# edwardyehuang/iSeg

Hardware: AMD Instinct MI355X
Metric: train_images_per_sec (ConvNeXt-T+ASPP 512x512 crop, fwd+bwd+AdamW, whole job) (higher is better)
Workload: dtype bf16

## Files before the change

### include/iseg_hip.h

```cpp
#ifndef ISEG_HIP_H
#define ISEG_HIP_H

#include <stddef.h>
#include <stdint.h>

#ifdef __cplusplus
extern "C" {
#endif

#ifndef ISEG_HIP_STREAM_T
#define ISEG_HIP_STREAM_T
typedef struct ihipStream_t* iseg_stream_t;
#endif

#define ISEG_STATUS_OK 0
#define ISEG_STATUS_ARG (-1)
#define ISEG_STATUS_HIP (-2)
#define ISEG_STATUS_UNSUPPORTED (-3)
#define ISEG_STATUS_WORKSPACE (-4)

#define ISEG_DTYPE_F32 0
#define ISEG_DTYPE_BF16 1

#define ISEG_ACT_NONE 0
// ... 484 lines not shown
int iseg_convnext_weight_prep_batched(const int64_t* table, int entries, int64_t max_elements, iseg_stream_t stream);
int iseg_convnext_mlp_fwd(const void* y2, const void* fw_tiled, const float* b1, const float* b2, const float* gamma,
                          const float* rowscale, int64_t rows_per_group, const void* residual, void* out, int64_t M, int C, int dtype,
                          iseg_stream_t stream);
int iseg_convnext_mlp_bwd(const void* y2, const void* dbr, const void* bw_tiled, const float* b1, void* g, void* dh, void* dy2,
                          int64_t M, int C, int dtype, iseg_stream_t stream);
int iseg_convnext_mlp_bwd_data(const void* y, const float* mean, const float* rstd, const float* ln_gamma, const float* ln_beta,
                               const void* dout, const float* rowscale, int64_t rows_per_group, const void* bw_tiled, const float* b1,
                               void* dy2, int64_t M, int C, int dtype, iseg_stream_t stream);

size_t iseg_convnext_mlp_bwd_data_ln_workspace_bytes(int64_t M, int C);
int iseg_convnext_mlp_bwd_data_ln(const void* y1, const float* mean, const float* rstd, const float* ln_gamma, const float* ln_beta,
                                  const void* dout, const float* rowscale, int64_t rows_per_group, const void* bw_tiled, const float* b1,
                                  void* dy1, float* dln_gamma, float* dln_beta, int64_t M, int C, int dtype, void* ws, size_t ws_bytes,
                                  iseg_stream_t stream);
int iseg_convnext_mlp_fwd_ln(const void* y1, const float* ln_gamma, const float* ln_beta, float eps, float* mean, float* rstd,
                             const void* fw_tiled, const float* b1, const float* b2, const float* gamma, const float* rowscale,
                             int64_t rows_per_group, const void* residual, void* out, int64_t M, int C, int dtype, iseg_stream_t stream);
size_t iseg_convnext_mlp_wgrad_workspace_bytes(int64_t M, int C);
int iseg_convnext_mlp_wgrad(const void* y, const float* mean, const float* rstd, const float* ln_gamma, const float* ln_beta,
                            const void* dout, const float* rowscale, int64_t rows_per_group, const void* bw_tiled, const float* b1,
                            const float* W2, const float* b2, const float* gamma, float* dW1, float* db1, float* dW2, float* db2,
                            float* dgamma, int64_t M, int C, int dtype, void* ws, size_t ws_bytes, iseg_stream_t stream);

#ifdef __cplusplus
}
#endif
#endif
```

### iseg_amd/_hip.py

```python
import ctypes as C
import os

_HERE = os.path.dirname(os.path.abspath(__file__))
LIB_PATH = os.path.join(_HERE, "lib", "libiseg_hip.so")

F32, BF16 = 0, 1
ACT_NONE, ACT_RELU, ACT_GELU, ACT_GELU_GRAD, ACT_RELU_GRAD, ACT_MUL_AUX, ACT_SIGMOID, ACT_SWISH = 0, 1, 2, 3, 4, 5, 6, 7


class HipLibraryMissing(RuntimeError):
    pass


class HipCallError(RuntimeError):
    pass


class GemmArgs(C.Structure):
    _fields_ = [
        ("A", C.c_void_p), ("lda", C.c_int64), ("a_kcontig", C.c_int),
        ("B", C.c_void_p), ("ldb", C.c_int64), ("b_kcontig", C.c_int),
        ("D", C.c_void_p), ("ldd", C.c_int64),
        ("M", C.c_int64), ("N", C.c_int64), ("K", C.c_int64),
        ("in_dtype", C.c_int), ("out_dtype", C.c_int),
# ... 233 lines not shown
    "iseg_conv2d_patch_fwd": (_i, [_p, _p, _p, _p, C.POINTER(ConvGeom), _i, _p, _z, _p]),
    "iseg_conv2d_patch_bwd_data": (_i, [_p, _p, _p, C.POINTER(ConvGeom), _i, _p, _z, _p]),
    "iseg_conv2d_patch_bwd_weight": (_i, [_p, _p, _p, _p, _i, C.POINTER(ConvGeom), _i, _p, _z, _p]),
    "iseg_conv2d_branches_supported": (_i, [C.POINTER(ConvBranches), _i]),
    "iseg_conv2d_branches_fwd": (_i, [_p, C.POINTER(ConvBranches), _i, _p, _z, _p]),
    "iseg_conv2d_branches_bwd_data": (_i, [C.POINTER(ConvBranches), _p, _p, _l, _i, _p, _z, _p]),
    "iseg_conv2d_branches_bwd_weight": (_i, [_p, C.POINTER(ConvBranches), _i, _i, _p, _z, _p]),
    "iseg_convnext_mlp_supported": (_i, [_i, _i]),
    "iseg_convnext_mlp_tiled_bytes": (_z, [_i, _i]),
    "iseg_convnext_mlp_prep": (_i, [_p, _p, _p, _p, _p, _i, _p]),
    "iseg_convnext_mlp_fwd": (_i, [_p, _p, _p, _p, _p, _p, _l, _p, _p, _l, _i, _i, _p]),
    "iseg_convnext_mlp_bwd": (_i, [_p, _p, _p, _p, _p, _p, _p, _l, _i, _i, _p]),
    "iseg_convnext_mlp_bwd_data": (_i, [_p, _p, _p, _p, _p, _p, _p, _l, _p, _p, _p, _l, _i, _i, _p]),
    "iseg_convnext_mlp_bwd_data_ln_workspace_bytes": (_z, [_l, _i]),
    "iseg_convnext_mlp_bwd_data_ln": (_i, [_p, _p, _p, _p, _p, _p, _p, _l, _p, _p, _p, _p, _p, _l, _i, _i, _p, _z, _p]),
    "iseg_convnext_weight_prep_batched": (_i, [_p, _i, _l, _p]),
    "iseg_convnext_mlp_fwd_ln": (_i, [_p, _p, _p, _f, _p, _p, _p, _p, _p, _p, _p, _l, _p, _p, _l, _i, _i, _p]),
    "iseg_convnext_mlp_wgrad_workspace_bytes": (_z, [_l, _i]),
    "iseg_convnext_mlp_wgrad": (_i, [_p, _p, _p, _p, _p, _p, _p, _l, _p, _p, _p, _p, _p, _p, _p, _p, _p, _p, _l, _i, _i, _p, _z, _p]),
    "iseg_sgd_momentum_step": (_i, [_p, _p, _p, _p, _p, _p, _p, _p, _f, _i, _p, _f, _p, _f, _l, _p]),
}

_lib = None


def lib():
    global _lib
    if _lib is None:
        if not os.path.exists(LIB_PATH):
            raise HipLibraryMissing(
# ... 27 lines not shown
```

### iseg_amd/csrc/mlp_fused.hip

```cpp
#include "common.h"
#include "iseg_hip.h"
#include "mlp_common.h"
#include <stdlib.h>

namespace {

typedef __attribute__((ext_vector_type(16))) float f32x16;
typedef __attribute__((address_space(3))) void* lds_void_ptr;
typedef const __attribute__((address_space(1))) void* glb_void_ptr;

constexpr int OUT_SLAB = 32 * 36 * 4;

template <int C, int SUB, int WAVES, int NIMG, int NSTAGES> struct MlpGeom {
    static constexpr int NS = NSTAGES;
    static constexpr int HID = 4 * C, KK = C / 16, CB = C / 32;
    static constexpr int IMG = C * 64;
    static constexpr int SLAB = NIMG * IMG;
    static constexpr int STAGE = SUB * SLAB;
    static constexpr int PIECES = STAGE / 1024;
    static constexpr int PLO = PIECES / WAVES, NHI = PIECES % WAVES, PHI = PLO + (NHI ? 1 : 0);
    static constexpr int NST = HID / (32 * SUB);
    static constexpr int RING = NS * STAGE > WAVES * OUT_SLAB ? NS * STAGE : WAVES * OUT_SLAB;
    static constexpr int LDS = RING + HID * 4;
    static_assert(C % 32 == 0 && STAGE % 1024 == 0 && HID % (32 * SUB) == 0 && PLO >= 1 && NST >= NS - 1 && NS >= 2 && LDS <= 160 * 1024, "geometry");
// ... 184 lines not shown
        for (int w = 0; w < 2; ++w) {
            auto sw = __builtin_amdgcn_permlane32_swap(d[4 * pr + w], d[4 * pr + 2 + w], false, false);
            d[4 * pr + w] = sw[0];
            d[4 * pr + 2 + w] = sw[1];
        }
    p0 = make_uint4(d[0], d[1], d[2], d[3]);
    p1 = make_uint4(d[4], d[5], d[6], d[7]);
}

template <int C, int SUB, int WAVES, int NSTAGES, bool STORE, bool LNB = false>
__global__ __launch_bounds__(64 * WAVES) void convnext_mlp_bwd_kernel(const bf16_t* __restrict__ Y, const bf16_t* __restrict__ D,
                                                                      const float* __restrict__ rowscale, int64_t rows_per_group,
                                                                      const void* __restrict__ BW, const float* __restrict__ b1,
                                                                      bf16_t* __restrict__ Gout, bf16_t* __restrict__ DHout,
                                                                      bf16_t* __restrict__ DY, int64_t M, MlpLayerNorm ln,
                                                                      float* __restrict__ ln_partials) {
    using G = MlpGeom<C, SUB, WAVES, 3, NSTAGES>;
    constexpr int HID = G::HID, KK = G::KK, CB = G::CB, IMG = G::IMG, SLAB = G::SLAB, STAGE = G::STAGE, NST = G::NST, NS = G::NS;
    constexpr int STORES = STORE ? 4 * SUB : 0;
    extern __shared__ __attribute__((aligned(1024))) char smem[];
    float* const b1s = reinterpret_cast<float*>(smem + G::RING);

    const int tid = threadIdx.x, lane = tid & 63, wid = tid >> 6;
    const int r = lane & 31, h = lane >> 5;
    const int64_t m0 = (int64_t)blockIdx.x * (32 * WAVES) + wid * 32;
    const bool active = m0 < M;

    bf16x8 yf[KK], df[KK];
    {
        int64_t row = m0 + r;
        row = row < M ? row : M - 1;
// ... 163 lines not shown
        }
    } else {
        float* const lnacc = reinterpret_cast<float*>(smem + WAVES * OUT_SLAB);
        float* const gam_s = lnacc + WAVES * 2 * C;
        const int64_t mr = m < M ? m : M - 1;
        bf16x8 yraw[CB][2];
#pragma unroll
        for (int cb = 0; cb < CB; ++cb) {
            yraw[cb][0] = *reinterpret_cast<const bf16x8*>(Y + mr * C + 32 * cb + 16 * eh);
            yraw[cb][1] = *reinterpret_cast<const bf16x8*>(Y + mr * C + 32 * cb + 16 * eh + 8);
        }
        const float mean = ln.mean[mr], rstd = ln.rstd[mr];
        for (int i = tid; i < WAVES * 2 * C; i += 64 * WAVES) lnacc[i] = 0.f;
        for (int i = tid; i < C; i += 64 * WAVES) gam_s[i] = ln.gamma[i];
        __syncthreads();
        const bool live = active && m < M;
        float s1 = 0.f, s2 = 0.f;
        auto xhat16 = [&](int cb, float* xh) {
#pragma unroll
            for (int u = 0; u < 8; ++u) {
                xh[u] = ((float)yraw[cb][0][u] - mean) * rstd;
                xh[8 + u] = ((float)yraw[cb][1][u] - mean) * rstd;
            }
        };
        auto gamma16 = [&](int c0, float* gm) {
#pragma unroll
            for (int i = 0; i < 4; ++i) {
                const float4 t = *reinterpret_cast<const float4*>(gam_s + c0 + 4 * i);
                gm[4 * i] = t.x, gm[4 * i + 1] = t.y, gm[4 * i + 2] = t.z, gm[4 * i + 3] = t.w;
            }
// ... 125 lines not shown
                   int64_t rows_per_group, const void* residual, void* out, int64_t M, const MlpLayerNorm& ln, hipStream_t s) {
    using G = MlpGeom<C, SUB, WAVES, 2, NSTAGES>;
    static const bool raised = [] {
        return hipFuncSetAttribute(reinterpret_cast<const void*>(&convnext_mlp_fwd_kernel<C, SUB, WAVES, NSTAGES>),
                                   hipFuncAttributeMaxDynamicSharedMemorySize, G::LDS) == hipSuccess;
    }();
    (void)raised;
    const int grid = (int)ceil_div64(M, 32 * WAVES);
    hipLaunchKernelGGL((convnext_mlp_fwd_kernel<C, SUB, WAVES, NSTAGES>), dim3(grid), dim3(64 * WAVES), G::LDS, s, (const bf16_t*)y2, FW, b1, b2, gamma, rowscale,
                       rows_per_group, (const bf16_t*)residual, (bf16_t*)out, M, ln);
    return iseg_check_launch("iseg_convnext_mlp_fwd");
}

template <int C, int SUB, int WAVES, int NSTAGES, bool STORE, bool LNB = false>
int launch_mlp_bwd(const void* y2, const void* dbr, const float* rowscale, int64_t rows_per_group, const void* BW, const float* b1, void* g,
                   void* dh, void* dy2, int64_t M, const MlpLayerNorm& ln, hipStream_t s, float* ln_partials = nullptr) {
    using G = MlpGeom<C, SUB, WAVES, 3, NSTAGES>;
    static_assert(!LNB || G::RING >= WAVES * OUT_SLAB + (WAVES * 2 + 1) * C * 4, "the column sums and gamma sit behind the epilogue slabs inside the ring");
    static const bool raised = [] {
        return hipFuncSetAttribute(reinterpret_cast<const void*>(&convnext_mlp_bwd_kernel<C, SUB, WAVES, NSTAGES, STORE, LNB>),
                                   hipFuncAttributeMaxDynamicSharedMemorySize, G::LDS) == hipSuccess;
    }();
    (void)raised;
    const int grid = (int)ceil_div64(M, 32 * WAVES);
    hipLaunchKernelGGL((convnext_mlp_bwd_kernel<C, SUB, WAVES, NSTAGES, STORE, LNB>), dim3(grid), dim3(64 * WAVES), G::LDS, s, (const bf16_t*)y2,
                       (const bf16_t*)dbr, rowscale, rows_per_group, BW, b1, (bf16_t*)g, (bf16_t*)dh, (bf16_t*)dy2, M, ln, ln_partials);
    return iseg_check_launch("iseg_convnext_mlp_bwd");
}

}

extern "C" int iseg_convnext_mlp_supported(int C, int dtype) {
    return dtype == ISEG_BF16 && (C == 96 || C == 192) ? 1 : 0;
}

extern "C" size_t iseg_convnext_mlp_tiled_bytes(int C, int backward) { return (size_t)(backward ? 3 : 2) * 4 * C * C * 2; }

extern "C" int iseg_convnext_mlp_prep(const float* W1, const float* W2, const float* gamma, void* fw_tiled, void* bw_tiled, int C,
                                      hipStream_t stream) {
    ISEG_REQUIRE(W1 && W2 && fw_tiled && C > 0 && C % 32 == 0, "iseg_convnext_mlp_prep: bad arguments");
    const int total = (bw_tiled ? 5 : 2) * 4 * C * C;
// ... 57 lines not shown
    ISEG_REQUIRE((((uintptr_t)y2 | (uintptr_t)dout | (uintptr_t)bw_tiled | (uintptr_t)b1 | (uintptr_t)dy2) & 15) == 0,
                 "iseg_convnext_mlp_bwd_data: operands must be 16-byte aligned");
    ISEG_REQUIRE(!mean || (rstd && ln_gamma && ln_beta && (((uintptr_t)ln_gamma | (uintptr_t)ln_beta) & 15) == 0),
                 "iseg_convnext_mlp_bwd_data: mean needs rstd and 16-byte aligned ln_gamma / ln_beta");
    const MlpLayerNorm ln{mean ? ln_gamma : nullptr, ln_beta, const_cast<float*>(mean), const_cast<float*>(rstd), 0.f};
    if (C == 96) return launch_mlp_bwd<96, 2, 8, 3, false>(y2, dout, rowscale, rows_per_group, bw_tiled, b1, nullptr, nullptr, dy2, M, ln, stream);
    return launch_mlp_bwd<192, 1, 4, 3, false>(y2, dout, rowscale, rows_per_group, bw_tiled, b1, nullptr, nullptr, dy2, M, ln, stream);
}

static int64_t mlp_bwd_blocks(int64_t M, int C) { return ceil_div64(M, 32 * (C == 96 ? 8 : 4)); }

extern "C" size_t iseg_convnext_mlp_bwd_data_ln_workspace_bytes(int64_t M, int C) {
    return (C == 96 || C == 192) && M > 0 ? (size_t)mlp_bwd_blocks(M, C) * 2 * C * sizeof(float) : 0;
}

extern "C" int iseg_convnext_mlp_bwd_data_ln(const void* y1, const float* mean, const float* rstd, const float* ln_gamma, const float* ln_beta,
                                             const void* dout, const float* rowscale, int64_t rows_per_group, const void* bw_tiled,
                                             const float* b1, void* dy1, float* dln_gamma, float* dln_beta, int64_t M, int C, int dtype,
                                             void* ws, size_t ws_bytes, hipStream_t stream) {
    ISEG_REQUIRE(dtype == ISEG_BF16 && (C == 96 || C == 192), "iseg_convnext_mlp_bwd_data_ln: bf16 storage with C = 96 or 192 only (C = %d, dtype = %d)", C, dtype);
    ISEG_REQUIRE(y1 && mean && rstd && ln_gamma && ln_beta && dout && bw_tiled && b1 && dy1 && dln_gamma && dln_beta && M > 0,
                 "iseg_convnext_mlp_bwd_data_ln: null operand or empty problem");
    ISEG_REQUIRE(!rowscale || rows_per_group > 0, "iseg_convnext_mlp_bwd_data_ln: rowscale needs rows_per_group > 0");
    ISEG_REQUIRE((((uintptr_t)y1 | (uintptr_t)dout | (uintptr_t)bw_tiled | (uintptr_t)b1 | (uintptr_t)dy1 | (uintptr_t)ln_gamma | (uintptr_t)ln_beta) & 15) == 0,
                 "iseg_convnext_mlp_bwd_data_ln: operands must be 16-byte aligned");
    const size_t need = iseg_convnext_mlp_bwd_data_ln_workspace_bytes(M, C);
    ISEG_NEED_WORKSPACE("iseg_convnext_mlp_bwd_data_ln", ws, ws_bytes, need);
    const MlpLayerNorm ln{ln_gamma, ln_beta, const_cast<float*>(mean), const_cast<float*>(rstd), 0.f};
    float* partials = (float*)ws;
    float* const arena = iseg_deferred_partials(need, dln_gamma, dln_beta, 1, stream);
    if (arena) partials = arena;
    const int rc = C == 96 ? launch_mlp_bwd<96, 2, 8, 3, false, true>(y1, dout, rowscale, rows_per_group, bw_tiled, b1, nullptr, nullptr, dy1, M, ln,
                                                                       stream, partials)
                           : launch_mlp_bwd<192, 1, 4, 3, false, true>(y1, dout, rowscale, rows_per_group, bw_tiled, b1, nullptr, nullptr, dy1, M, ln,
                                                                        stream, partials);
    if (rc != ISEG_OK) return rc;
    const int blocks = (int)mlp_bwd_blocks(M, C);
    if (arena) iseg_deferred_push(partials, blocks, 2 * C, 2 * C, dln_gamma, dln_beta, C, 1.f, stream);
    else launch_reduce_rows(partials, blocks, 2 * C, 0, 1, 2 * C, dln_gamma, dln_beta, C, 0, 1.f, 1, stream);
    return iseg_check_launch("iseg_convnext_mlp_bwd_data_ln");
}
```

### iseg_amd/csrc/mlp_wgrad.hip

```cpp
#include "common.h"
#include "iseg_hip.h"
#include "mlp_common.h"

namespace {

typedef __attribute__((address_space(3))) bf16x4* lds_bf16x4_ptr;

template <int C> struct WgGeom {
    static constexpr int WAVES = 8, NT = 64 * WAVES, RT = C > 96 ? 32 : 64;
    static constexpr int HID = 4 * C, KS = C / 32, CBS = C / 16;
    static constexpr int NHG = HID / (16 * WAVES);
    static constexpr int STRIDE = (((2 * C + 223) / 256) * 256 + 32) / 2;
    static constexpr int TILE = RT * STRIDE;
    static constexpr int CPR = C / 8;
    static constexpr int RG = (NT / CPR) >= 32 ? 32 : 16;
    static constexpr int NLOAD = CPR * RG, RPT = RT / RG;
    static constexpr int LDS = 2 * 2 * TILE * 2;
    static constexpr int IMG = C * 64, SLAB = 3 * IMG;
    static_assert(C % 32 == 0 && HID % (16 * WAVES) == 0 && NLOAD <= NT && RT % RG == 0 && LDS <= 160 * 1024, "geometry");
};

__device__ __forceinline__ f32x4 mfma16(const bf16x8& a, const bf16x8& b, const f32x4& c) {
    return __builtin_amdgcn_mfma_f32_16x16x32_bf16(a, b, c, 0, 0, 0);
}

__device__ __forceinline__ bf16x8 tr_frag(const bf16_t* rows, int stride, int cb, int lane) {
    const int q = lane >> 4, qq = (lane >> 2) & 3, p = lane & 3;
    const bf16_t* a0 = rows + (4 * q + qq) * stride + 16 * cb + 4 * p;
    const bf16x4 lo = __builtin_amdgcn_ds_read_tr16_b64_v4bf16((lds_bf16x4_ptr)(a0));
    const bf16x4 hi = __builtin_amdgcn_ds_read_tr16_b64_v4bf16((lds_bf16x4_ptr)(a0 + 16 * stride));
    bf16x8 f;
#pragma unroll
    for (int i = 0; i < 4; ++i) {
        f[i] = lo[i];
        f[4 + i] = hi[i];
    }
    return f;
}

template <int C>
__global__ __launch_bounds__(512) void convnext_mlp_wgrad_kernel(const bf16_t* __restrict__ Y, const float* __restrict__ mean,
                                                                 const float* __restrict__ rstd, const float* __restrict__ ln_gamma,
                                                                 const float* __restrict__ ln_beta, const bf16_t* __restrict__ D,
                                                                 const float* __restrict__ rowscale, int64_t rows_per_group,
                                                                 const void* __restrict__ BW, const float* __restrict__ b1,
                                                                 float* __restrict__ part, int64_t M, int64_t rows_per_chunk, int nchunk) {
    using G = WgGeom<C>;
    constexpr int HID = G::HID, KS = G::KS, CBS = G::CBS, STRIDE = G::STRIDE, TILE = G::TILE, RT = G::RT, RG = G::RG, RPT = G::RPT, CPR = G::CPR;
    extern __shared__ __attribute__((aligned(16))) char smem[];
    bf16_t* const tiles = reinterpret_cast<bf16_t*>(smem);

    const int wg = blockIdx.x, xcd = wg & 7, idx = wg >> 3;
    const int hg = idx % G::NHG, chunk = (idx / G::NHG) * 8 + xcd;
    if (chunk >= nchunk) return;
    const int tid = threadIdx.x, lane = tid & 63, wid = tid >> 6;
    const int li = lane & 15, q = lane >> 4;
    const int hid0 = (hg * G::WAVES + wid) * 16;
    const int64_t r_begin = (int64_t)chunk * rows_per_chunk;
    const int64_t r_end = r_begin + rows_per_chunk < M ? r_begin + rows_per_chunk : M;
    const int ntiles = (int)((r_end - r_begin + RT - 1) / RT);

    bf16x8 w1f[KS], w3f[KS];
    {
        const char* slab = (const char*)BW + (int64_t)(hid0 >> 5) * G::SLAB;
        const int row = (hid0 & 16) + li;
#pragma unroll
        for (int ks = 0; ks < KS; ++ks) {
            const int off = (2 * ks + (q >> 1)) * 1024 + mlp_frag_offset(row, q & 1);
            w1f[ks] = *reinterpret_cast<const bf16x8*>(slab + off);
            w3f[ks] = *reinterpret_cast<const bf16x8*>(slab + G::IMG + off);
        }
// ... 7 lines not shown
    for (int u = 0; u < 8; ++u) s_acc[u] = 0.f;
    bf16x8 ry[RPT], rd[RPT];
    float rmean[RPT], rrstd[RPT];
    bool rok[RPT];

    auto issue = [&](int t) {
        const bool live = t < ntiles;
        const int tt = live ? t : ntiles - 1;
#pragma unroll
        for (int i = 0; i < RPT; ++i) {
            const int64_t row = r_begin + (int64_t)tt * RT + rg + RG * i;
            const bool ok = live && loader && row < r_end;
            const int64_t rr = row < r_end ? row : r_begin;
            ry[i] = *reinterpret_cast<const bf16x8*>(Y + rr * C + 8 * cpos);
            rd[i] = *reinterpret_cast<const bf16x8*>(D + rr * C + 8 * cpos);
            if (mean) {
                rmean[i] = mean[rr];
                rrstd[i] = rstd[rr];
            }
            rok[i] = ok;
        }
    };
    auto commit = [&](int t, int buf) {
        const int64_t row0 = r_begin + (int64_t)(t < ntiles ? t : ntiles - 1) * RT;
        const float rs = rowscale ? rowscale[row0 / rows_per_group] : 1.f;
        bf16_t* const ty = tiles + (buf * 2 + 0) * TILE;
        bf16_t* const td = tiles + (buf * 2 + 1) * TILE;
        float lg[8], lb[8];
        if (mean) {
            load8<float>(ln_gamma + 8 * cpos, lg);
            load8<float>(ln_beta + 8 * cpos, lb);
        }
#pragma unroll
        for (int i = 0; i < RPT; ++i) {
            const int r = rg + RG * i;
            bf16x8 y = ry[i], d = rd[i];
            if (!rok[i]) {
#pragma unroll
                for (int u = 0; u < 8; ++u) {
                    y[u] = (bf16_t)0.f;
                    d[u] = (bf16_t)0.f;
                }
            }
            if (mean && rok[i]) {
#pragma unroll
                for (int u = 0; u < 8; ++u) y[u] = (bf16_t)iseg_ln_apply((float)y[u], rmean[i], rrstd[i], lg[u], lb[u]);
            }
            if (rowscale) {
#pragma unroll
                for (int u = 0; u < 8; ++u) d[u] = (bf16_t)((float)d[u] * rs);
            }
#pragma unroll
            for (int u = 0; u < 8; ++u) s_acc[u] += (float)d[u];
            if (loader) {
                *reinterpret_cast<bf16x8*>(ty + r * STRIDE + 8 * cpos) = y;
                *reinterpret_cast<bf16x8*>(td + r * STRIDE + 8 * cpos) = d;
            }
        }
    };

    f32x4 zacc[CBS], wacc[CBS];
#pragma unroll
    for (int cb = 0; cb < CBS; ++cb)
// ... 169 lines not shown
        const int hid = h0 + threadIdx.x;
        db1[hid] += rec[2 * plane + hid];
    }
}

template <int C> int rows_per_chunk_for(int64_t M, int* nchunk) {
    using G = WgGeom<C>;
    const int target = 8 * (32 / G::NHG);
    int64_t rpc = (M + target - 1) / target;
    rpc = (rpc + 63) / 64 * 64;
    if (rpc < 256) rpc = 256;
    *nchunk = (int)((M + rpc - 1) / rpc);
    return (int)rpc;
}

template <int C>
int launch_wgrad(const void* y, const float* mean, const float* rstd, const float* lng, const float* lnb, const void* d, const float* rowscale,
                 int64_t rows_per_group, const void* BW, const float* b1, float* ws, int64_t M, hipStream_t s) {
    using G = WgGeom<C>;
    int nchunk;
    const int rpc = rows_per_chunk_for<C>(M, &nchunk);
    static const bool raised = [] {
        return hipFuncSetAttribute(reinterpret_cast<const void*>(&convnext_mlp_wgrad_kernel<C>), hipFuncAttributeMaxDynamicSharedMemorySize,
                                   G::LDS) == hipSuccess;
    }();
    (void)raised;
    float* part = ws;
    const int grid = 8 * G::NHG * ((nchunk + 7) / 8);
    hipLaunchKernelGGL((convnext_mlp_wgrad_kernel<C>), dim3(grid), dim3(G::NT), G::LDS, s, (const bf16_t*)y, mean, rstd, lng, lnb, (const bf16_t*)d,
                       rowscale, rows_per_group, BW, b1, part, M, (int64_t)rpc, nchunk);
    return iseg_check_launch("iseg_convnext_mlp_wgrad");
}

size_t wgrad_ws_floats(int C, int64_t M, int* nchunk_out) {
    int nchunk;
    if (C == 96) rows_per_chunk_for<96>(M, &nchunk);
    else rows_per_chunk_for<192>(M, &nchunk);
    if (nchunk_out) *nchunk_out = nchunk;
    const size_t rec = 2 * 4 * (size_t)C * C + 4 * C + C;
    return (size_t)(nchunk + 1) * rec + (size_t)(4 * C / FIN_ROWS) * C;
}

}

// ... 6 lines not shown
                                       const void* dout, const float* rowscale, int64_t rows_per_group, const void* bw_tiled, const float* b1,
                                       const float* W2, const float* b2, const float* gamma, float* dW1, float* db1, float* dW2, float* db2,
                                       float* dgamma, int64_t M, int C, int dtype, void* ws, size_t ws_bytes, hipStream_t stream) {
    ISEG_REQUIRE(dtype == ISEG_BF16 && (C == 96 || C == 192), "iseg_convnext_mlp_wgrad: bf16 storage with C = 96 or 192 only (C = %d, dtype = %d)", C, dtype);
    ISEG_REQUIRE(y && dout && bw_tiled && b1 && W2 && b2 && dW1 && db1 && dW2 && db2 && M > 0, "iseg_convnext_mlp_wgrad: null operand or empty problem");
    ISEG_REQUIRE(!gamma || dgamma, "iseg_convnext_mlp_wgrad: gamma needs dgamma");
    ISEG_REQUIRE(!mean || (rstd && ln_gamma && ln_beta), "iseg_convnext_mlp_wgrad: mean needs rstd, ln_gamma and ln_beta");
    ISEG_REQUIRE(!rowscale || (rows_per_group > 0 && rows_per_group % 64 == 0),
                 "iseg_convnext_mlp_wgrad: the row factor must be constant inside 64-row tiles (rows_per_group = %lld)", (long long)rows_per_group);
    ISEG_REQUIRE((((uintptr_t)y | (uintptr_t)dout | (uintptr_t)bw_tiled | (uintptr_t)ln_gamma | (uintptr_t)ln_beta) & 15) == 0,
                 "iseg_convnext_mlp_wgrad: operands must be 16-byte aligned");
    int nchunk;
    const size_t need = wgrad_ws_floats(C, M, &nchunk) * sizeof(float);
    ISEG_NEED_WORKSPACE("iseg_convnext_mlp_wgrad", ws, ws_bytes, need);
    float* const wsf = (float*)ws;
    int rc = C == 96 ? launch_wgrad<96>(y, mean, rstd, ln_gamma, ln_beta, dout, rowscale, rows_per_group, bw_tiled, b1, wsf, M, stream)
                     : launch_wgrad<192>(y, mean, rstd, ln_gamma, ln_beta, dout, rowscale, rows_per_group, bw_tiled, b1, wsf, M, stream);
    if (rc != ISEG_OK) return rc;
    const int HID = 4 * C;
    const int64_t rec = 2 * (int64_t)HID * C + HID + C;
    float* part = wsf;
    float* sum = part + (int64_t)nchunk * rec;
    float* gpart_ws = sum + rec;
    launch_reduce_rows(part, nchunk, rec, 0, 1, rec, sum, nullptr, rec, 0, 1.f, 0, stream);
    const int P = HID / FIN_ROWS;
    float* gpart = gpart_ws;
    float* arena = nullptr;
    if (gamma) {
        arena = iseg_deferred_partials((size_t)P * C * sizeof(float), dgamma, nullptr, 1, stream);
        if (arena) gpart = arena;
    }
    hipLaunchKernelGGL(convnext_mlp_wgrad_finish_kernel, dim3(C / 32, HID / FIN_ROWS), dim3(256), 0, stream, sum, W2, b2, gamma,
// ... 8 lines not shown
```

### iseg_amd/functional.py

```python
import os

import torch
from torch.autograd import Function

from . import kernels as K
from . import nn
from . import dist


def _grad(p):
    if p.grad is None:
        p.grad = torch.zeros_like(p.data)
    return p.grad


def _c(t):
    return t if t.is_contiguous() else t.contiguous()


def _rows2d(t):
    C = t.shape[-1]
    if t.is_contiguous():
        return t.reshape(-1, C), C
    per16 = 16 // t.element_size()
# ... 208 lines not shown
        M = x2.shape[0]
        rpg = M // rowscale.shape[0] if rowscale is not None else 0
        fw, bw = nn.mlp_tiled(W1, W2, None)
        out, mean, rstd = K.convnext_mlp_fwd_ln(x2, ln_gamma.data, ln_beta.data, eps, fw, b1.data, b2.data, None, rowscale, rpg, x2)
        ctx.params, ctx.rpg = (ln_gamma, ln_beta, W1, b1, W2, b2), rpg
        ctx.save_for_backward(x2, mean, rstd, bw, rowscale)
        return out.reshape(x.shape)

    @staticmethod
    def backward(ctx, dout):
        x2, mean, rstd, bw, rowscale = ctx.saved_tensors
        ln_gamma, ln_beta, W1, b1, W2, b2 = ctx.params
        M, C = x2.shape
        do2 = _c(dout).reshape(M, C)
        ln = (mean, rstd, ln_gamma.data, ln_beta.data)
        dx = None
        if ctx.needs_input_grad[0]:
            dln = K.convnext_mlp_bwd_data_ln(x2, do2, bw, b1.data, ln, _grad(ln_gamma), _grad(ln_beta), rowscale, ctx.rpg)
            dx = K.axpby(do2, dln, 1.0, 1.0, out=dln).reshape(dout.shape)
        else:
            K.convnext_mlp_bwd_data_ln(x2, do2, bw, b1.data, ln, _grad(ln_gamma), _grad(ln_beta), rowscale, ctx.rpg)
        K.convnext_mlp_wgrad(x2, do2, bw, b1.data, W2.data, b2.data, None, _grad(W1), _grad(b1), _grad(W2), _grad(b2), None, rowscale, ctx.rpg, ln=ln)
        dist.grads_ready(ln_gamma, ln_beta, W1, b1, W2, b2)
        return (dx,) + (None,) * 8


def ln_mlp_residual_supported(x, params, drop_path_mask=None):
    ln_gamma, ln_beta, W1, b1, W2, b2 = params
    C = x.shape[-1]
    if any(p is None for p in params) or not K.convnext_mlp_supported(C, x.dtype) or C not in (96, 192):
        return False
    if tuple(W1.shape) != (C, 4 * C) or tuple(W2.shape) != (4 * C, C):
        return False
    if not all(p.requires_grad for p in params) and torch.is_grad_enabled() and (x.requires_grad or any(p.requires_grad for p in params)):
        return False
    rows = x.numel() // C
    return drop_path_mask is None or (rows % drop_path_mask.shape[0] == 0 and (rows // drop_path_mask.shape[0]) % 64 == 0)


# ... 1234 lines not shown
        ctx.p, ctx.dil, ctx.pad = p, dil, pad
        ctx.save_for_backward(xc, y1, y2, mean, rstd, h, g if grad else None, dp_mask)
        return out.reshape(N, H, W, C)

    @staticmethod
    def backward(ctx, dout):
        xc, y1, y2, mean, rstd, h, g, dp_mask = ctx.saved_tensors
        p, dil, pad = ctx.p, ctx.dil, ctx.pad
        N, H, W, C = xc.shape
        M = N * H * W
        Kk = p.dw_kernel.shape[0]
        do2 = _c(dout).reshape(M, C)
        cdt = xc.dtype
        if ctx.ln_on_load:
            y1m, ln = y1.reshape(M, C), (mean, rstd, p.ln_gamma.data, p.ln_beta.data)
            dy1 = K.convnext_mlp_bwd_data_ln(y1m, do2, h, p.b1.data, ln, _grad(p.ln_gamma), _grad(p.ln_beta), dp_mask, H * W)
            K.convnext_mlp_wgrad(y1m, do2, h, p.b1.data, p.w2.data, p.b2.data, p.gamma.data if p.gamma is not None else None,
                                 _grad(p.w1), _grad(p.b1), _grad(p.w2), _grad(p.b2), _grad(p.gamma) if p.gamma is not None else None, dp_mask,
                                 H * W, ln=ln)
            del h
        else:
            dy2 = _ConvNeXtBlockFn._mlp_backward_with_hidden(ctx, p, do2, y2, h, g, dp_mask, H, W, C, M, cdt, xc)
            del h, g
            dy1 = K.layernorm_bwd(dy2, y1.reshape(M, C), p.ln_gamma.data, mean, rstd, _grad(p.ln_gamma), _grad(p.ln_beta))
        dy1 = dy1.reshape(N, H, W, C)
        K.dwconv2d_bwd_weight(xc, dy1, _grad(p.dw_kernel).reshape(Kk * Kk, C), _grad(p.dw_bias), Kk, dil, pad, pad)
        dx = None
        if ctx.needs_input_grad[0]:
            padb = (Kk - 1) * dil - pad
            dx = K.dwconv2d(dy1, p.dw_kernel.data.reshape(Kk * Kk, C), None, Kk, dil, padb, padb, flip=True, add=_c(dout))
        dist.grads_ready(p.dw_kernel, p.dw_bias, p.ln_gamma, p.ln_beta, p.w1, p.b1, p.w2, p.b2, p.gamma)
        return (dx,) + (None,) * 12

    @staticmethod
    def _mlp_backward_with_hidden(ctx, p, do2, y2, h, g, dp_mask, H, W, C, M, cdt, xc):
# ... 1319 lines not shown
```

### iseg_amd/kernels.py

```python
import contextlib
import ctypes as C

import torch

from . import _hip
from ._hip import F32, BF16, ACT_NONE, ACT_RELU, ACT_GELU, ACT_GELU_GRAD, ACT_RELU_GRAD, ACT_MUL_AUX, ACT_SIGMOID, ACT_SWISH, GemmArgs

_DT = {torch.float32: F32, torch.bfloat16: BF16}


def dt(t):
    try:
        return _DT[t.dtype if isinstance(t, torch.Tensor) else t]
    except KeyError:
        raise TypeError(f"iseg_amd kernels support float32 and bfloat16 storage, got {t.dtype if isinstance(t, torch.Tensor) else t}")


def ptr(t):
    return None if t is None else t.data_ptr()


_DEVICE_INDEX = [None]


# ... 302 lines not shown
    mean, rstd, lng, lnb = ln if ln is not None else (None, None, None, None)
    _hip.call("iseg_convnext_mlp_bwd_data", ptr(y), ptr(mean), ptr(rstd), ptr(lng), ptr(lnb), ptr(dout), ptr(rowscale), int(rows_per_group),
              ptr(bw_tiled), ptr(b1), ptr(dy2), M, Cc, dt(y), stream())
    return dy2


def convnext_mlp_bwd_data_ln(y1, dout, bw_tiled, b1, ln, dln_gamma, dln_beta, rowscale=None, rows_per_group=0):
    _require_cuda(y1, dout, bw_tiled, dln_gamma, dln_beta)
    M, Cc = y1.shape
    dy1 = torch.empty((M, Cc), dtype=y1.dtype, device=y1.device)
    mean, rstd, lng, lnb = ln
    need = _hip.lib().iseg_convnext_mlp_bwd_data_ln_workspace_bytes(M, Cc)
    ws, wsb = workspace(need, y1.device)
    _hip.call("iseg_convnext_mlp_bwd_data_ln", ptr(y1), ptr(mean), ptr(rstd), ptr(lng), ptr(lnb), ptr(dout), ptr(rowscale), int(rows_per_group),
              ptr(bw_tiled), ptr(b1), ptr(dy1), ptr(dln_gamma), ptr(dln_beta), M, Cc, dt(y1), ptr(ws), wsb, stream())
    return dy1


def convnext_mlp_wgrad(y, dout, bw_tiled, b1, W2, b2, gamma, dW1, db1, dW2, db2, dgamma, rowscale=None, rows_per_group=0, ln=None):
    _require_cuda(y, dout, bw_tiled)
    M, Cc = y.shape
    need = _hip.lib().iseg_convnext_mlp_wgrad_workspace_bytes(M, Cc)
    ws, wsb = workspace(need, y.device)
    mean, rstd, lng, lnb = ln if ln is not None else (None, None, None, None)
    _hip.call("iseg_convnext_mlp_wgrad", ptr(y), ptr(mean), ptr(rstd), ptr(lng), ptr(lnb), ptr(dout), ptr(rowscale), int(rows_per_group),
              ptr(bw_tiled), ptr(b1), ptr(W2), ptr(b2), ptr(gamma), ptr(dW1), ptr(db1), ptr(dW2), ptr(db2), ptr(dgamma), M, Cc, dt(y), ptr(ws),
              wsb, stream())


def layernorm_fwd(x2d, gamma, beta, eps, save_stats=True):
# ... 1458 lines not shown
```

Baseline: 2055.

## Emit LayerNorm output and scaled grad from bwd-data kernel for wgrad reuse

The fused MLP backward-data kernel, which already applies LayerNorm and drop-path rowscale on load, now optionally writes the normalized activations (y2) and the row-scaled output gradient (dbr) to global memory. The weight-gradient kernel then consumes these precomputed operands through a new GIVEN template path that skips recomputing LayerNorm and rowscale per tile. This removes duplicated normalization work in wgrad. In exchange it adds two extra M×C bf16 writes and reads plus temporary allocations, and wgrad now always runs even when the input grad is not needed, which it did before too.

```diff
diff --git a/include/iseg_hip.h b/include/iseg_hip.h
--- a/include/iseg_hip.h
+++ b/include/iseg_hip.h
@@ -522,6 +522,10 @@
                                   const void* dout, const float* rowscale, int64_t rows_per_group, const void* bw_tiled, const float* b1,
                                   void* dy1, float* dln_gamma, float* dln_beta, int64_t M, int C, int dtype, void* ws, size_t ws_bytes,
                                   iseg_stream_t stream);
+int iseg_convnext_mlp_bwd_data_ln_ops(const void* y1, const float* mean, const float* rstd, const float* ln_gamma, const float* ln_beta,
+                                      const void* dout, const float* rowscale, int64_t rows_per_group, const void* bw_tiled, const float* b1,
+                                      void* dy1, float* dln_gamma, float* dln_beta, void* y2_out, void* dbr_out, int64_t M, int C, int dtype,
+                                      void* ws, size_t ws_bytes, iseg_stream_t stream);
 int iseg_convnext_mlp_fwd_ln(const void* y1, const float* ln_gamma, const float* ln_beta, float eps, float* mean, float* rstd,
                              const void* fw_tiled, const float* b1, const float* b2, const float* gamma, const float* rowscale,
                              int64_t rows_per_group, const void* residual, void* out, int64_t M, int C, int dtype, iseg_stream_t stream);
diff --git a/iseg_amd/_hip.py b/iseg_amd/_hip.py
--- a/iseg_amd/_hip.py
+++ b/iseg_amd/_hip.py
@@ -271,6 +271,7 @@
     "iseg_convnext_mlp_bwd_data": (_i, [_p, _p, _p, _p, _p, _p, _p, _l, _p, _p, _p, _l, _i, _i, _p]),
     "iseg_convnext_mlp_bwd_data_ln_workspace_bytes": (_z, [_l, _i]),
     "iseg_convnext_mlp_bwd_data_ln": (_i, [_p, _p, _p, _p, _p, _p, _p, _l, _p, _p, _p, _p, _p, _l, _i, _i, _p, _z, _p]),
+    "iseg_convnext_mlp_bwd_data_ln_ops": (_i, [_p, _p, _p, _p, _p, _p, _p, _l, _p, _p, _p, _p, _p, _p, _p, _l, _i, _i, _p, _z, _p]),
     "iseg_convnext_weight_prep_batched": (_i, [_p, _i, _l, _p]),
     "iseg_convnext_mlp_fwd_ln": (_i, [_p, _p, _p, _f, _p, _p, _p, _p, _p, _p, _p, _l, _p, _p, _l, _i, _i, _p]),
     "iseg_convnext_mlp_wgrad_workspace_bytes": (_z, [_l, _i]),
diff --git a/iseg_amd/csrc/mlp_fused.hip b/iseg_amd/csrc/mlp_fused.hip
--- a/iseg_amd/csrc/mlp_fused.hip
+++ b/iseg_amd/csrc/mlp_fused.hip
@@ -222,7 +222,8 @@
                                                                       const void* __restrict__ BW, const float* __restrict__ b1,
                                                                       bf16_t* __restrict__ Gout, bf16_t* __restrict__ DHout,
                                                                       bf16_t* __restrict__ DY, int64_t M, MlpLayerNorm ln,
-                                                                      float* __restrict__ ln_partials) {
+                                                                      float* __restrict__ ln_partials, bf16_t* __restrict__ Y2out,
+                                                                      bf16_t* __restrict__ DBRout) {
     using G = MlpGeom<C, SUB, WAVES, 3, NSTAGES>;
     constexpr int HID = G::HID, KK = G::KK, CB = G::CB, IMG = G::IMG, SLAB = G::SLAB, STAGE = G::STAGE, NST = G::NST, NS = G::NS;
     constexpr int STORES = STORE ? 4 * SUB : 0;
@@ -416,6 +417,17 @@
         for (int i = tid; i < WAVES * 2 * C; i += 64 * WAVES) lnacc[i] = 0.f;
         for (int i = tid; i < C; i += 64 * WAVES) gam_s[i] = ln.gamma[i];
         __syncthreads();
+        if (row_ok) {
+            const int64_t o = (m0 + r) * C + 8 * h;
+            if (Y2out) {
+#pragma unroll
+                for (int kk = 0; kk < KK; ++kk) *reinterpret_cast<bf16x8*>(Y2out + o + 16 * kk) = yf[kk];
+            }
+            if (DBRout) {
+#pragma unroll
+                for (int kk = 0; kk < KK; ++kk) *reinterpret_cast<bf16x8*>(DBRout + o + 16 * kk) = df[kk];
+            }
+        }
         const bool live = active && m < M;
         float s1 = 0.f, s2 = 0.f;
         auto xhat16 = [&](int cb, float* xh) {
@@ -571,7 +583,8 @@
 
 template <int C, int SUB, int WAVES, int NSTAGES, bool STORE, bool LNB = false>
 int launch_mlp_bwd(const void* y2, const void* dbr, const float* rowscale, int64_t rows_per_group, const void* BW, const float* b1, void* g,
-                   void* dh, void* dy2, int64_t M, const MlpLayerNorm& ln, hipStream_t s, float* ln_partials = nullptr) {
+                   void* dh, void* dy2, int64_t M, const MlpLayerNorm& ln, hipStream_t s, float* ln_partials = nullptr, void* y2_out = nullptr,
+                   void* dbr_out = nullptr) {
     using G = MlpGeom<C, SUB, WAVES, 3, NSTAGES>;
     static_assert(!LNB || G::RING >= WAVES * OUT_SLAB + (WAVES * 2 + 1) * C * 4, "the column sums and gamma sit behind the epilogue slabs inside the ring");
     static const bool raised = [] {
@@ -581,7 +594,8 @@
     (void)raised;
     const int grid = (int)ceil_div64(M, 32 * WAVES);
     hipLaunchKernelGGL((convnext_mlp_bwd_kernel<C, SUB, WAVES, NSTAGES, STORE, LNB>), dim3(grid), dim3(64 * WAVES), G::LDS, s, (const bf16_t*)y2,
-                       (const bf16_t*)dbr, rowscale, rows_per_group, BW, b1, (bf16_t*)g, (bf16_t*)dh, (bf16_t*)dy2, M, ln, ln_partials);
+                       (const bf16_t*)dbr, rowscale, rows_per_group, BW, b1, (bf16_t*)g, (bf16_t*)dh, (bf16_t*)dy2, M, ln, ln_partials,
+                       (bf16_t*)y2_out, (bf16_t*)dbr_out);
     return iseg_check_launch("iseg_convnext_mlp_bwd");
 }
 
@@ -669,29 +683,49 @@
     return (C == 96 || C == 192) && M > 0 ? (size_t)mlp_bwd_blocks(M, C) * 2 * C * sizeof(float) : 0;
 }
 
-extern "C" int iseg_convnext_mlp_bwd_data_ln(const void* y1, const float* mean, const float* rstd, const float* ln_gamma, const float* ln_beta,
-                                             const void* dout, const float* rowscale, int64_t rows_per_group, const void* bw_tiled,
-                                             const float* b1, void* dy1, float* dln_gamma, float* dln_beta, int64_t M, int C, int dtype,
-                                             void* ws, size_t ws_bytes, hipStream_t stream) {
-    ISEG_REQUIRE(dtype == ISEG_BF16 && (C == 96 || C == 192), "iseg_convnext_mlp_bwd_data_ln: bf16 storage with C = 96 or 192 only (C = %d, dtype = %d)", C, dtype);
+namespace {
+
+int mlp_bwd_data_ln(const char* who, const void* y1, const float* mean, const float* rstd, const float* ln_gamma, const float* ln_beta, const void* dout,
+                    const float* rowscale, int64_t rows_per_group, const void* bw_tiled, const float* b1, void* dy1, float* dln_gamma,
+                    float* dln_beta, void* y2_out, void* dbr_out, int64_t M, int C, int dtype, void* ws, size_t ws_bytes, hipStream_t stream) {
+    ISEG_REQUIRE(dtype == ISEG_BF16 && (C == 96 || C == 192), "%s: bf16 storage with C = 96 or 192 only (C = %d, dtype = %d)", who, C, dtype);
     ISEG_REQUIRE(y1 && mean && rstd && ln_gamma && ln_beta && dout && bw_tiled && b1 && dy1 && dln_gamma && dln_beta && M > 0,
-                 "iseg_convnext_mlp_bwd_data_ln: null operand or empty problem");
-    ISEG_REQUIRE(!rowscale || rows_per_group > 0, "iseg_convnext_mlp_bwd_data_ln: rowscale needs rows_per_group > 0");
-    ISEG_REQUIRE((((uintptr_t)y1 | (uintptr_t)dout | (uintptr_t)bw_tiled | (uintptr_t)b1 | (uintptr_t)dy1 | (uintptr_t)ln_gamma | (uintptr_t)ln_beta) & 15) == 0,
-                 "iseg_convnext_mlp_bwd_data_ln: operands must be 16-byte aligned");
+                 "%s: null operand or empty problem", who);
+    ISEG_REQUIRE(!rowscale || rows_per_group > 0, "%s: rowscale needs rows_per_group > 0", who);
+    ISEG_REQUIRE((((uintptr_t)y1 | (uintptr_t)dout | (uintptr_t)bw_tiled | (uintptr_t)b1 | (uintptr_t)dy1 | (uintptr_t)ln_gamma | (uintptr_t)ln_beta |
+                   (uintptr_t)y2_out | (uintptr_t)dbr_out) & 15) == 0, "%s: operands must be 16-byte aligned", who);
     const size_t need = iseg_convnext_mlp_bwd_data_ln_workspace_bytes(M, C);
-    ISEG_NEED_WORKSPACE("iseg_convnext_mlp_bwd_data_ln", ws, ws_bytes, need);
+    ISEG_NEED_WORKSPACE(who, ws, ws_bytes, need);
     const MlpLayerNorm ln{ln_gamma, ln_beta, const_cast<float*>(mean), const_cast<float*>(rstd), 0.f};
     float* partials = (float*)ws;
     float* const arena = iseg_deferred_partials(need, dln_gamma, dln_beta, 1, stream);
     if (arena) partials = arena;
     const int rc = C == 96 ? launch_mlp_bwd<96, 2, 8, 3, false, true>(y1, dout, rowscale, rows_per_group, bw_tiled, b1, nullptr, nullptr, dy1, M, ln,
-                                                                       stream, partials)
+                                                                       stream, partials, y2_out, dbr_out)
                            : launch_mlp_bwd<192, 1, 4, 3, false, true>(y1, dout, rowscale, rows_per_group, bw_tiled, b1, nullptr, nullptr, dy1, M, ln,
-                                                                        stream, partials);
+                                                                        stream, partials, y2_out, dbr_out);
     if (rc != ISEG_OK) return rc;
     const int blocks = (int)mlp_bwd_blocks(M, C);
     if (arena) iseg_deferred_push(partials, blocks, 2 * C, 2 * C, dln_gamma, dln_beta, C, 1.f, stream);
     else launch_reduce_rows(partials, blocks, 2 * C, 0, 1, 2 * C, dln_gamma, dln_beta, C, 0, 1.f, 1, stream);
-    return iseg_check_launch("iseg_convnext_mlp_bwd_data_ln");
-}
+    return iseg_check_launch(who);
+}
+
+}
+
+extern "C" int iseg_convnext_mlp_bwd_data_ln(const void* y1, const float* mean, const float* rstd, const float* ln_gamma, const float* ln_beta,
+                                             const void* dout, const float* rowscale, int64_t rows_per_group, const void* bw_tiled,
+                                             const float* b1, void* dy1, float* dln_gamma, float* dln_beta, int64_t M, int C, int dtype,
+                                             void* ws, size_t ws_bytes, hipStream_t stream) {
+    return mlp_bwd_data_ln("iseg_convnext_mlp_bwd_data_ln", y1, mean, rstd, ln_gamma, ln_beta, dout, rowscale, rows_per_group, bw_tiled, b1, dy1,
+                           dln_gamma, dln_beta, nullptr, nullptr, M, C, dtype, ws, ws_bytes, stream);
+}
+
+extern "C" int iseg_convnext_mlp_bwd_data_ln_ops(const void* y1, const float* mean, const float* rstd, const float* ln_gamma, const float* ln_beta,
+                                                 const void* dout, const float* rowscale, int64_t rows_per_group, const void* bw_tiled,
+                                                 const float* b1, void* dy1, float* dln_gamma, float* dln_beta, void* y2_out, void* dbr_out,
+                                                 int64_t M, int C, int dtype, void* ws, size_t ws_bytes, hipStream_t stream) {
+    ISEG_REQUIRE(!dbr_out || rowscale, "iseg_convnext_mlp_bwd_data_ln_ops: dbr_out needs rowscale (without one dbr is dout itself)");
+    return mlp_bwd_data_ln("iseg_convnext_mlp_bwd_data_ln_ops", y1, mean, rstd, ln_gamma, ln_beta, dout, rowscale, rows_per_group, bw_tiled, b1, dy1,
+                           dln_gamma, dln_beta, y2_out, dbr_out, M, C, dtype, ws, ws_bytes, stream);
+}
diff --git a/iseg_amd/csrc/mlp_wgrad.hip b/iseg_amd/csrc/mlp_wgrad.hip
--- a/iseg_amd/csrc/mlp_wgrad.hip
+++ b/iseg_amd/csrc/mlp_wgrad.hip
@@ -38,7 +38,7 @@
     return f;
 }
 
-template <int C>
+template <int C, bool GIVEN>
 __global__ __launch_bounds__(512) void convnext_mlp_wgrad_kernel(const bf16_t* __restrict__ Y, const float* __restrict__ mean,
                                                                  const float* __restrict__ rstd, const float* __restrict__ ln_gamma,
                                                                  const float* __restrict__ ln_beta, const bf16_t* __restrict__ D,
@@ -55,6 +55,7 @@
     if (chunk >= nchunk) return;
     const int tid = threadIdx.x, lane = tid & 63, wid = tid >> 6;
     const int li = lane & 15, q = lane >> 4;
+    const bool ln_on = !GIVEN && mean != nullptr, rs_on = !GIVEN && rowscale != nullptr;
     const int hid0 = (hg * G::WAVES + wid) * 16;
     const int64_t r_begin = (int64_t)chunk * rows_per_chunk;
     const int64_t r_end = r_begin + rows_per_chunk < M ? r_begin + rows_per_chunk : M;
@@ -92,7 +93,7 @@
             const int64_t rr = row < r_end ? row : r_begin;
             ry[i] = *reinterpret_cast<const bf16x8*>(Y + rr * C + 8 * cpos);
             rd[i] = *reinterpret_cast<const bf16x8*>(D + rr * C + 8 * cpos);
-            if (mean) {
+            if (ln_on) {
                 rmean[i] = mean[rr];
                 rrstd[i] = rstd[rr];
             }
@@ -101,11 +102,11 @@
     };
     auto commit = [&](int t, int buf) {
         const int64_t row0 = r_begin + (int64_t)(t < ntiles ? t : ntiles - 1) * RT;
-        const float rs = rowscale ? rowscale[row0 / rows_per_group] : 1.f;
+        const float rs = rs_on ? rowscale[row0 / rows_per_group] : 1.f;
         bf16_t* const ty = tiles + (buf * 2 + 0) * TILE;
         bf16_t* const td = tiles + (buf * 2 + 1) * TILE;
         float lg[8], lb[8];
-        if (mean) {
+        if (ln_on) {
             load8<float>(ln_gamma + 8 * cpos, lg);
             load8<float>(ln_beta + 8 * cpos, lb);
         }
@@ -120,11 +121,11 @@
                     d[u] = (bf16_t)0.f;
                 }
             }
-            if (mean && rok[i]) {
+            if (ln_on && rok[i]) {
 #pragma unroll
                 for (int u = 0; u < 8; ++u) y[u] = (bf16_t)iseg_ln_apply((float)y[u], rmean[i], rrstd[i], lg[u], lb[u]);
             }
-            if (rowscale) {
+            if (rs_on) {
 #pragma unroll
                 for (int u = 0; u < 8; ++u) d[u] = (bf16_t)((float)d[u] * rs);
             }
@@ -324,20 +325,20 @@
     return (int)rpc;
 }
 
-template <int C>
+template <int C, bool GIVEN>
 int launch_wgrad(const void* y, const float* mean, const float* rstd, const float* lng, const float* lnb, const void* d, const float* rowscale,
                  int64_t rows_per_group, const void* BW, const float* b1, float* ws, int64_t M, hipStream_t s) {
     using G = WgGeom<C>;
     int nchunk;
     const int rpc = rows_per_chunk_for<C>(M, &nchunk);
     static const bool raised = [] {
-        return hipFuncSetAttribute(reinterpret_cast<const void*>(&convnext_mlp_wgrad_kernel<C>), hipFuncAttributeMaxDynamicSharedMemorySize,
+        return hipFuncSetAttribute(reinterpret_cast<const void*>(&convnext_mlp_wgrad_kernel<C, GIVEN>), hipFuncAttributeMaxDynamicSharedMemorySize,
                                    G::LDS) == hipSuccess;
     }();
     (void)raised;
     float* part = ws;
     const int grid = 8 * G::NHG * ((nchunk + 7) / 8);
-    hipLaunchKernelGGL((convnext_mlp_wgrad_kernel<C>), dim3(grid), dim3(G::NT), G::LDS, s, (const bf16_t*)y, mean, rstd, lng, lnb, (const bf16_t*)d,
+    hipLaunchKernelGGL((convnext_mlp_wgrad_kernel<C, GIVEN>), dim3(grid), dim3(G::NT), G::LDS, s, (const bf16_t*)y, mean, rstd, lng, lnb, (const bf16_t*)d,
                        rowscale, rows_per_group, BW, b1, part, M, (int64_t)rpc, nchunk);
     return iseg_check_launch("iseg_convnext_mlp_wgrad");
 }
@@ -374,8 +375,9 @@
     const size_t need = wgrad_ws_floats(C, M, &nchunk) * sizeof(float);
     ISEG_NEED_WORKSPACE("iseg_convnext_mlp_wgrad", ws, ws_bytes, need);
     float* const wsf = (float*)ws;
-    int rc = C == 96 ? launch_wgrad<96>(y, mean, rstd, ln_gamma, ln_beta, dout, rowscale, rows_per_group, bw_tiled, b1, wsf, M, stream)
-                     : launch_wgrad<192>(y, mean, rstd, ln_gamma, ln_beta, dout, rowscale, rows_per_group, bw_tiled, b1, wsf, M, stream);
+    const bool given = !mean && !rowscale;
+    auto launch = C == 96 ? (given ? launch_wgrad<96, true> : launch_wgrad<96, false>) : (given ? launch_wgrad<192, true> : launch_wgrad<192, false>);
+    int rc = launch(y, mean, rstd, ln_gamma, ln_beta, dout, rowscale, rows_per_group, bw_tiled, b1, wsf, M, stream);
     if (rc != ISEG_OK) return rc;
     const int HID = 4 * C;
     const int64_t rec = 2 * (int64_t)HID * C + HID + C;
diff --git a/iseg_amd/functional.py b/iseg_amd/functional.py
--- a/iseg_amd/functional.py
+++ b/iseg_amd/functional.py
@@ -246,15 +246,20 @@
         M, C = x2.shape
         do2 = _c(dout).reshape(M, C)
         ln = (mean, rstd, ln_gamma.data, ln_beta.data)
+        y2, dbr = _mlp_row_operands(x2, do2, rowscale)
+        dln = K.convnext_mlp_bwd_data_ln_ops(x2, do2, bw, b1.data, ln, _grad(ln_gamma), _grad(ln_beta), rowscale, ctx.rpg, y2,
+                                             dbr if rowscale is not None else None)
+        K.convnext_mlp_wgrad(y2, dbr, bw, b1.data, W2.data, b2.data, None, _grad(W1), _grad(b1), _grad(W2), _grad(b2), None)
+        del y2, dbr
         dx = None
         if ctx.needs_input_grad[0]:
-            dln = K.convnext_mlp_bwd_data_ln(x2, do2, bw, b1.data, ln, _grad(ln_gamma), _grad(ln_beta), rowscale, ctx.rpg)
             dx = K.axpby(do2, dln, 1.0, 1.0, out=dln).reshape(dout.shape)
-        else:
-            K.convnext_mlp_bwd_data_ln(x2, do2, bw, b1.data, ln, _grad(ln_gamma), _grad(ln_beta), rowscale, ctx.rpg)
-        K.convnext_mlp_wgrad(x2, do2, bw, b1.data, W2.data, b2.data, None, _grad(W1), _grad(b1), _grad(W2), _grad(b2), None, rowscale, ctx.rpg, ln=ln)
         dist.grads_ready(ln_gamma, ln_beta, W1, b1, W2, b2)
         return (dx,) + (None,) * 8
+
+
+def _mlp_row_operands(y1, dout, rowscale):
+    return torch.empty_like(y1), torch.empty_like(dout) if rowscale is not None else dout
 
 
 def ln_mlp_residual_supported(x, params, drop_path_mask=None):
@@ -1519,11 +1524,12 @@
         cdt = xc.dtype
         if ctx.ln_on_load:
             y1m, ln = y1.reshape(M, C), (mean, rstd, p.ln_gamma.data, p.ln_beta.data)
-            dy1 = K.convnext_mlp_bwd_data_ln(y1m, do2, h, p.b1.data, ln, _grad(p.ln_gamma), _grad(p.ln_beta), dp_mask, H * W)
-            K.convnext_mlp_wgrad(y1m, do2, h, p.b1.data, p.w2.data, p.b2.data, p.gamma.data if p.gamma is not None else None,
-                                 _grad(p.w1), _grad(p.b1), _grad(p.w2), _grad(p.b2), _grad(p.gamma) if p.gamma is not None else None, dp_mask,
-                                 H * W, ln=ln)
-            del h
+            y2s, dbr = _mlp_row_operands(y1m, do2, dp_mask)
+            dy1 = K.convnext_mlp_bwd_data_ln_ops(y1m, do2, h, p.b1.data, ln, _grad(p.ln_gamma), _grad(p.ln_beta), dp_mask, H * W, y2s,
+                                                 dbr if dp_mask is not None else None)
+            K.convnext_mlp_wgrad(y2s, dbr, h, p.b1.data, p.w2.data, p.b2.data, p.gamma.data if p.gamma is not None else None,
+                                 _grad(p.w1), _grad(p.b1), _grad(p.w2), _grad(p.b2), _grad(p.gamma) if p.gamma is not None else None)
+            del h, y2s, dbr
         else:
             dy2 = _ConvNeXtBlockFn._mlp_backward_with_hidden(ctx, p, do2, y2, h, g, dp_mask, H, W, C, M, cdt, xc)
             del h, g
diff --git a/iseg_amd/kernels.py b/iseg_amd/kernels.py
--- a/iseg_amd/kernels.py
+++ b/iseg_amd/kernels.py
@@ -340,6 +340,21 @@
     ws, wsb = workspace(need, y1.device)
     _hip.call("iseg_convnext_mlp_bwd_data_ln", ptr(y1), ptr(mean), ptr(rstd), ptr(lng), ptr(lnb), ptr(dout), ptr(rowscale), int(rows_per_group),
               ptr(bw_tiled), ptr(b1), ptr(dy1), ptr(dln_gamma), ptr(dln_beta), M, Cc, dt(y1), ptr(ws), wsb, stream())
+    return dy1
+
+
+def convnext_mlp_bwd_data_ln_ops(y1, dout, bw_tiled, b1, ln, dln_gamma, dln_beta, rowscale=None, rows_per_group=0, y2_out=None, dbr_out=None):
+    _require_cuda(y1, dout, bw_tiled, dln_gamma, dln_beta)
+    M, Cc = y1.shape
+    for t in (y2_out, dbr_out):
+        if t is not None and (tuple(t.shape) != (M, Cc) or t.dtype != y1.dtype or not t.is_contiguous()):
+            raise ValueError("convnext_mlp_bwd_data_ln_ops: y2_out / dbr_out must be contiguous [M, C] tensors of the operand type")
+    dy1 = torch.empty((M, Cc), dtype=y1.dtype, device=y1.device)
+    mean, rstd, lng, lnb = ln
+    need = _hip.lib().iseg_convnext_mlp_bwd_data_ln_workspace_bytes(M, Cc)
+    ws, wsb = workspace(need, y1.device)
+    _hip.call("iseg_convnext_mlp_bwd_data_ln_ops", ptr(y1), ptr(mean), ptr(rstd), ptr(lng), ptr(lnb), ptr(dout), ptr(rowscale), int(rows_per_group),
+              ptr(bw_tiled), ptr(b1), ptr(dy1), ptr(dln_gamma), ptr(dln_beta), ptr(y2_out), ptr(dbr_out), M, Cc, dt(y1), ptr(ws), wsb, stream())
     return dy1
 
 
```

Result: faster. 2084 (median of 6 runs) (+1.4%).
